# carsonswope/3d-beats

Hardware: AMD Instinct MI355X
Metric: classified Mpix/s on 848x480 depth frames (4 trees, depth 20); % of the bounding roofline level (roofline.bound; HBM: roofline.hbm_frac) (higher is better)
Workload: dtype f32

## Files before the change

3d-beats_amd/_lib.py:

```python
import ctypes
import os
import threading
import warnings

from . import _build

_c_int, _c_float, _c_void_p, _c_size_t = ctypes.c_int, ctypes.c_float, ctypes.c_void_p, ctypes.c_size_t

SIGNATURES = {
    "rdf_eval_forest": (_c_int, [_c_void_p, _c_int, _c_int, _c_int, _c_void_p, _c_int, _c_int, _c_int,
                                 _c_void_p, _c_int, _c_void_p, _c_int, _c_float, _c_void_p]),
    "rdf_eval_tree": (_c_int, [_c_void_p, _c_int, _c_int, _c_int, _c_void_p, _c_int, _c_int, _c_void_p,
                               _c_void_p]),
    "rdf_composite": (_c_int, [_c_void_p, _c_int, _c_int, _c_int, _c_void_p, _c_int, _c_void_p, _c_void_p,
                               _c_void_p]),
    "rdf_layered_run": (_c_int, [_c_void_p, _c_int, _c_int, _c_int, _c_void_p, _c_void_p, _c_void_p, _c_void_p, _c_void_p,
                                 _c_void_p, _c_void_p, _c_void_p, _c_void_p, _c_void_p, _c_int, _c_void_p, _c_void_p,
                                 _c_int, _c_float, _c_void_p]),
    "rdf_layered_run_hand": (_c_int, [_c_void_p, _c_int, _c_int, _c_int, _c_void_p, _c_void_p, _c_void_p, _c_void_p, _c_void_p,
                                      _c_void_p, _c_void_p, _c_void_p, _c_void_p, _c_void_p, _c_int, _c_void_p, _c_void_p,
                                      _c_int, _c_float, _c_int, _c_void_p, _c_int, _c_void_p, _c_void_p]),
    "rdf_layered_run_hand_batch": (_c_int, [_c_void_p, _c_int, _c_int, _c_int, _c_int, _c_void_p, _c_void_p, _c_void_p, _c_void_p,
                                            _c_void_p, _c_void_p, _c_void_p, _c_void_p, _c_void_p, _c_void_p, _c_int, _c_void_p,
                                            _c_void_p, _c_int, _c_float, _c_int, _c_void_p, _c_int, _c_void_p, _c_void_p]),
# ... 76 lines not shown
    "rdf_ipc_export": (_c_int, [_c_void_p, _c_void_p]),
    "rdf_ipc_open": (_c_int, [_c_void_p, _c_void_p]),
    "rdf_ipc_close": (_c_int, [_c_void_p]),
    "rdf_memcpy_device_async": (_c_int, [_c_void_p, _c_void_p, _c_size_t, _c_void_p]),
    "rdf_debug_fat_kernel": (_c_int, [_c_int, ctypes.c_uint64, _c_void_p, _c_void_p]),
    "rdf_debug_floor_i32": (_c_int, [_c_void_p, _c_void_p, _c_size_t, _c_void_p]),
    "rdf_debug_div_f32": (_c_int, [_c_void_p, _c_void_p, _c_void_p, _c_size_t, _c_void_p]),
    "rdf_set_lds_budget_bytes": (None, [_c_int]),
    "rdf_set_block_threads": (None, [_c_int]),
    "rdf_set_scheduler": (None, [_c_int]),
    "rdf_set_compaction": (None, [_c_int]),
    "rdf_set_halo": (None, [_c_int]),
    "rdf_set_lds_levels": (None, [_c_int]),
    "rdf_set_tree_waves": (None, [_c_int]),
    "rdf_set_stage_vec": (None, [_c_int]),
    "rdf_set_group": (None, [_c_int]),
    "rdf_set_layers_one_launch": (None, [_c_int]),
    "rdf_set_rows_per_wave": (None, [_c_int]),
    "rdf_set_force_exact": (None, [_c_int]),
    "rdf_set_last_level_table": (None, [_c_int]),
    "rdf_set_deep_from": (None, [_c_int]),
    "rdf_set_fold": (None, [_c_int]),
    "rdf_set_plain_levels": (None, [_c_int]),
    "rdf_event_create": (_c_int, [ctypes.POINTER(_c_void_p)]),
    "rdf_event_record": (_c_int, [_c_void_p, _c_void_p]),
    "rdf_event_synchronize": (_c_int, [_c_void_p]),
    "rdf_event_elapsed_ms": (_c_int, [_c_void_p, _c_void_p, ctypes.POINTER(_c_float)]),
    "rdf_event_destroy": (_c_int, [_c_void_p]),
    "rdf_stream_synchronize": (_c_int, [_c_void_p]),
    "rdf_abi_version": (_c_int, []),
    "rdf_build_id": (ctypes.c_char_p, []),
    "rdf_error_string": (ctypes.c_char_p, [_c_int]),
}

ABI_VERSION = 5


class StereoConfig(ctypes.Structure):
    _fields_ = [("fb16", ctypes.c_int32), ("fbp16", ctypes.c_int32), ("max_disparity", ctypes.c_int32),
                ("dot_threshold", ctypes.c_uint32), ("pattern_seed", ctypes.c_uint32), ("ambient", ctypes.c_int32),
                ("ir_noise_amp", ctypes.c_int32), ("census_margin", ctypes.c_int32), ("uniqueness", ctypes.c_int32),
                ("lr_max", ctypes.c_int32), ("dq_min", ctypes.c_int32)]


class DepthFilterConfig(ctypes.Structure):
    _fields_ = [(name, ctypes.c_int32) for name in ("spatial_radius", "spatial_delta", "temporal", "temporal_alpha", "temporal_delta",
# ... 152 lines not shown
```

3d-beats_amd/csrc/rdf_hip.hip:

```cpp

#include <hip/hip_runtime.h>
#include <stdint.h>
#include <stdio.h>
#include <stdlib.h>
#include <string.h>
#include <time.h>
#include <unistd.h>

#include <algorithm>
#include <array>
#include <atomic>
#include <mutex>
#include <utility>
#include <vector>

#include "../../include/rdf_hip.h"
#include "rdf_device.hpp"
#include "rdf_host_state.hpp"
#include "rdf_launch_plan.hpp"

namespace {

constexpr uint32_t kFlagLeftLeaf = 1u, kFlagRightLeaf = 2u, kFlagExact = 4u;
using rdf_host::kSchedSlots;
using rdf_host::kGraphSlots;

constexpr uint32_t kStealFrom = 2;
constexpr uint32_t kXcdQueuesFrom = 64;
__device__ unsigned int g_sched[kSchedSlots + kGraphSlots][kSchedWords];

__device__ __forceinline__ uint32_t child_flags(float l, float r)
{
    return ((l >= -1.0f && l < 0.0f) ? 0u : kFlagLeftLeaf) | ((r >= -1.0f && r < 0.0f) ? 0u : kFlagRightLeaf);
}

__device__ __forceinline__ bool int_offset_ok(float a)
{
    const uint32_t b = __float_as_uint(a);
    return (b << 1) == 0u || (((b >> 23) & 0xFFu) - 40u) <= 107u;
}

__device__ __forceinline__ uint32_t guarded_payload(uint32_t byte)
{
    return (byte & 0xFFu) | ((~byte & 0x80u) << 1);
}

__device__ __forceinline__ int thresh_to_int(float t)
{
    if (t != t) return -65535;
    const float c = fminf(fmaxf(__builtin_ceilf(t), -65535.0f), 65536.0f);
    return (int)c;
}
// ... 85 lines not shown
    const uint32_t role = NL > 1 ? blockIdx.x % NL : 0u;
    const uint32_t block_id = NL > 1 ? blockIdx.x / NL : blockIdx.x, n_blocks = NL > 1 ? gridDim.x / NL : gridDim.x;
    const EvalArgs &a = ka.l[role];
    extern __shared__ __align__(16) unsigned char lds_raw[];
    uint16_t *lds_tile = reinterpret_cast<uint16_t *>(lds_raw);
    uint4 *lds_nodes = reinterpret_cast<uint4 *>(lds_raw + a.lds_nodes_off);
    uint32_t *s_tile = reinterpret_cast<uint32_t *>(lds_raw + a.lds_mail_off);
    uint16_t *px_list = reinterpret_cast<uint16_t *>(lds_raw + a.lds_list_off);

    const int tid = threadIdx.x;
    const int lane = tid & 63;
    const int K = a.lds_levels;
    const uint32_t nodes_lds = (1u << K) - 1u;
    constexpr uint32_t kWaves = BLOCK / 64;
    const int rows_per_wave = a.rows_per_wave;
    const uint32_t wave = (uint32_t)tid >> 6;
    const uint32_t tw_T = TW ? (uint32_t)a.T : 1u;
    const uint32_t tw_row = TW ? wave / tw_T : 0u, tw_tree = TW ? wave - tw_row * tw_T : 0u;
    const uint32_t tile_rows = TW ? (kWaves / tw_T) * (uint32_t)rows_per_wave : kWaves * (uint32_t)rows_per_wave;

    const uint32_t lds_pitch = 1u << K;
    constexpr bool kLastLevelTable = PACKED && CMAX == 4 && !TW;
    constexpr bool kPlainLevels = PACKED && !STATS && !TW && !DEEP && NL == 1 && BLOCK == 512 && CMAX == 4 && GROUP == 4 && !COMPACT;
    bool last_from_table = false;
    if (kLastLevelTable && a.last_level) {
        const uint2 t = *reinterpret_cast<const uint2 *>(a.last_level + (((size_t)a.T << (a.D - 1)) << 2));
        last_from_table = t.x == 0u && t.y >= a.last_level_min;
    }
    constexpr int kDeepLast = CMAX == 4 ? 2 : 1;
    bool deep_on = false;
    if (DEEP && a.deep) {
        const uint2 t = *reinterpret_cast<const uint2 *>(a.deep + ((deep_total_lines(a.T, a.D, a.cpad) + 1u) << 3));
        deep_on = (uint32_t)a.deep_from >= t.x && t.y == 0u;
    }
    if (DEEP && deep_on) last_from_table = false;
    const int walk_levels = (DEEP && deep_on) ? a.deep_from : last_from_table ? a.D - 1 : a.D;
    for (uint32_t i = tid; i < (uint32_t)a.T * lds_pitch; i += BLOCK) {
        const uint32_t k = i >> K, h = i & (lds_pitch - 1u);
        if (h == 0u) {
            if (K > 0) lds_nodes[i] = make_uint4(0u, 0u, 0u, 0u);
            continue;
        }
        if (PACKED) {
            lds_nodes[i] = reinterpret_cast<const uint4 *>(a.packed16)[((size_t)k << a.D) + h];
        } else {
            const float *p = a.forest + ((size_t)k * (size_t)a.nodes + (h - 1u)) * (size_t)a.E;
// ... 21 lines not shown
        return (active && (!prev_active || prev != line)) ? 1u : 0u;
    };
    const char *depth_b = reinterpret_cast<const char *>(a.depth);
    const uint32_t xcc = (uint32_t)__builtin_amdgcn_s_getreg(20 | (31 << 11)) & 7u;
    const uint32_t q_static = a.q_static ? a.q_static : n_blocks;
    const uint32_t q_blocks = a.q_blocks ? a.q_blocks : n_blocks;
    const uint32_t queued = a.n_tiles > q_static ? a.n_tiles - q_static : 0u;

    struct TilePlace { uint32_t img, x0, y0, fold, col_shift; bool narrow; };
    auto place_tile = [&](uint32_t tile) -> TilePlace {
        const uint32_t tiles_wide = a.tiles_x * a.tiles_y;
        const uint32_t tiles_per_img = tiles_wide + a.tiles_y_n;
        TilePlace p;
        p.img = tile / tiles_per_img;
        const uint32_t trem = tile - p.img * tiles_per_img;
        p.narrow = trem >= tiles_wide;
        const uint32_t ty = p.narrow ? trem - tiles_wide : trem / a.tiles_x;
        const uint32_t tx = p.narrow ? a.tiles_x : trem - ty * a.tiles_x;
        p.fold = p.narrow ? a.fold : 1u;
        p.col_shift = p.narrow ? (a.fold == 4u ? 4u : 5u) : 6u;
        p.x0 = tx * 64u, p.y0 = ty * tile_rows * p.fold;
        return p;
    };
    auto rows_have_pixels = [&](const TilePlace &p, uint32_t first, uint32_t step, bool store_fails) -> bool {
        const uint32_t lane_col = (uint32_t)lane & ((1u << p.col_shift) - 1u), lane_row = (uint32_t)lane >> p.col_shift;
        const uint32_t lx = p.x0 + lane_col;
        const int y_last = min(a.Hl, (int)(p.y0 + tile_rows * p.fold)) - 1;
        const uint32_t img_boff = (p.img * a.per_img_d) << 1, img_loff = p.img * a.per_img_l;
        const uint32_t dy = step * p.fold;
        uint32_t ly = p.y0 + first * p.fold + lane_row;
        uint32_t seen = 0u;
        if ((int)lx < a.Wl) {
#pragma clang loop unroll(disable)
            for (uint32_t trow = first; trow < tile_rows; trow += 4u * step, ly += 4u * dy) {
                uint32_t i[4], d[4];
#pragma unroll
                for (uint32_t k = 0; k < 4u; ++k) {
                    const uint32_t y = (uint32_t)min((int)(ly + k * dy), y_last);
                    i[k] = img_loff + y * (uint32_t)a.Wl + lx;
                    d[k] = *reinterpret_cast<const uint16_t *>(
                        depth_b + (img_boff + ((__umul24(y * (uint32_t)a.r, (uint32_t)a.W) + lx * (uint32_t)a.r) << 1)));
                }
                if (a.filter_class != -1) {
                    uint32_t f[4];
#pragma unroll
                    for (uint32_t k = 0; k < 4u; ++k) f[k] = a.filter[i[k]];
#pragma unroll
                    for (uint32_t k = 0; k < 4u; ++k) d[k] = (int)f[k] == a.filter_class ? d[k] : 0u;
                }
#pragma unroll
                for (uint32_t k = 0; k < 4u; ++k) {
                    d[k] = (d[k] + 1u) & 0xFFFFu;
                    seen = max(seen, d[k]);
                    if (store_fails && d[k] <= 1u) a.labels[i[k]] = (uint16_t)kNoPixel;
                }
            }
        }
        return seen > 1u;
    };
    auto fill_tile = [&](const TilePlace &p) {
        const uint32_t lane_col = (uint32_t)lane & ((1u << p.col_shift) - 1u), lane_row = (uint32_t)lane >> p.col_shift;
        const int lx = (int)(p.x0 + lane_col);
#pragma clang loop vectorize(disable) unroll(disable)
        for (uint32_t trow = 0; trow < tile_rows; ++trow) {
            const int ly = (int)(p.y0 + trow * p.fold + lane_row);
            if (ly < a.Hl && lx < a.Wl) a.labels[p.img * a.per_img_l + (uint32_t)ly * (uint32_t)a.Wl + (uint32_t)lx] = (uint16_t)kNoPixel;
        }
    };
    auto pull_tile = [&](uint32_t after, uint32_t &q_empty) -> uint32_t {
        if (!a.sched) return after + n_blocks < a.n_tiles ? after + n_blocks : a.n_tiles;
        uint32_t t = a.n_tiles;
        if (q_static < kXcdQueuesFrom) {
            const uint32_t got = atomicAdd(a.sched, 1u);
            if (got < queued) t = q_static + got;
        } else {
            const uint32_t reach = (((block_id >> 3) & 15u) == 0u || queued >= 2u * q_static || a.q_helper) ? 7u : kStealFrom;
            for (uint32_t k = 0; k <= reach; ++k) {
                const uint32_t q = (xcc + k) & 7u;
                if ((q_empty >> q) & 1u) continue;
                const uint32_t lo = (uint32_t)(((unsigned long long)queued * q) >> 3);
                const uint32_t hi = (uint32_t)(((unsigned long long)queued * (q + 1u)) >> 3);
                const uint32_t got = lo < hi ? atomicAdd(a.sched + q * kSchedStride, 1u) : hi;
                if (lo < hi && got < hi - lo) { t = q_static + lo + got; break; }
                q_empty |= 1u << q;
            }
        }
        return t;
    };
    const bool more_tiles = a.sched ? queued != 0u : block_id + n_blocks < a.n_tiles;
    bool scout = !TW && a.sched && a.q_helper && wave == 0u;
    uint32_t q_empty = 0u;
    uint32_t tile = block_id;

    for (uint32_t it = 0;; ++it) {
        const bool own_tile = it == 0u && !(a.sched && a.q_helper);
        if (!own_tile && !more_tiles) break;
        if (TW) {
            if (!own_tile && tid == 0) s_tile[it & 1u] = pull_tile(tile, q_empty);
        } else {
            if (own_tile && a.check_empty) __syncthreads();
            if (scout || (own_tile && a.check_empty)) {
                uint32_t t = tile;
                q_empty = s_tile[6];
                for (;;) {
                    if (!own_tile) {
                        if (lane == 0) t = pull_tile(t, q_empty);
                        t = (uint32_t)__builtin_amdgcn_readfirstlane((int)t);
                    }
                    if (t >= a.n_tiles || !a.check_empty) break;
                    const TilePlace p = place_tile(t);
                    const bool any = (p.narrow ? a.tw_n : a.tw) <= 0 ||
                                     __any(rows_have_pixels(p, own_tile ? wave : 0u, own_tile ? kWaves : 1u, own_tile && a.fill_untouched));
                    if (own_tile) {
                        if (any && lane == 0) s_tile[2] = 1u;
                        break;
                    }
                    if (any) break;
                    if (a.fill_untouched) fill_tile(p);
                }
                if (!own_tile && lane == 0) {
                    s_tile[it & 1u] = t;
                    s_tile[6] = q_empty;
                }
            }
            scout = false;
        }
        __syncthreads();
        if (!own_tile) {
            tile = (uint32_t)__builtin_amdgcn_readfirstlane((int)s_tile[it & 1u]);
            if (!TW && tid == 0) s_tile[4u + ((it + 1u) & 1u)] = 0u;
        }
        if (tile >= a.n_tiles) break;
        if (!TW && own_tile && a.check_empty && s_tile[2] == 0u) {
            scout = wave == 0u;
            continue;
        }
        const TilePlace tp = place_tile(tile);
        const uint32_t img = tp.img;
        const bool narrow = tp.narrow;
        const uint32_t fold = tp.fold, col_shift = tp.col_shift;
        const uint32_t lane_col = (uint32_t)lane & ((1u << col_shift) - 1u), lane_row = (uint32_t)lane >> col_shift;
        const uint32_t x0 = tp.x0, y0 = tp.y0;
        const int lx = (int)(x0 + lane_col);
        const uint32_t img_boff = (img * a.per_img_d) << 1;
        const uint32_t img_loff = img * a.per_img_l;
        const int tx0 = (int)x0 * a.r - (narrow ? a.halo_xn : a.halo);
        const int ty0 = (int)y0 * a.r - a.halo;
        const int tw = narrow ? a.tw_n : a.tw, th = narrow ? a.th_n : a.th, twp = narrow ? a.twp_n : a.twp;
        const uint32_t stage_tw8 = narrow ? a.stage_tw8_n : a.stage_tw8, stage_magic = narrow ? a.stage_magic_n : a.stage_magic;

        const TileCtx pc = {depth_b + img_boff,
                            (uint32_t)tw * 2u, (uint32_t)th, (uint32_t)twp * 2u, (uint32_t)a.W * 2u, (uint32_t)a.H,
// ... 75 lines not shown
            my_rank[sub] = (uint32_t)__popcll(b & ((1ull << lane) - 1ull));
            my_valid |= ok ? 1u << sub : 0u;
        }
        uint32_t n_valid = 64u * tile_rows;
        if (compact) {
            __syncthreads();
            n_valid = 0u;
            uint32_t my_base[kMaxRowsPerWave];
            for (uint32_t row = 0; row < tile_rows; ++row) {
#pragma unroll
                for (int sub = 0; sub < kMaxRowsPerWave; ++sub)
                    if (row == (uint32_t)sub * kWaves + wave) my_base[sub] = n_valid;
                n_valid += s_cnt[row];
            }
#pragma unroll
            for (int sub = 0; sub < kMaxRowsPerWave; ++sub) {
                if (sub >= rows_per_wave) break;
                if ((my_valid >> sub) & 1u)
                    px_list[my_base[sub] + my_rank[sub]] = (uint16_t)((((uint32_t)sub * kWaves + wave) << 6) | (uint32_t)lane);
            }
            __syncthreads();
        }

        constexpr uint32_t kDone = 0x80000000u, kIdle = 0xFFFFFFFFu;
        auto add_leaf_pdf = [&](uint32_t hk, int tree, int c0, float (&pdf)[CMAX]) -> bool {
            if (STATS && c0 == 0)
                st_leaf += lines_of((int)hk < 0 && hk != kIdle, PACKED ? (hk & ~kDone) * (uint32_t)(a.cpad * 4) : ((hk & ~kDone) >> 1) * (uint32_t)a.E * 4u);
            if (!((int)hk < 0 && hk != kIdle)) return false;
            const uint32_t leaf = (hk & ~kDone) - 2u;
            if (PACKED) {
                const float4 *pp = reinterpret_cast<const float4 *>(a.packed_pdf) +
                    (((((size_t)tree) << a.D) + (leaf >> 1) + 1u) * 2u + (leaf & 1u)) * (size_t)(a.cpad >> 2) +
                    (size_t)(c0 >> 2);
#pragma unroll
                for (int c = 0; c < CMAX; c += 4) {
                    if (c0 + c < a.cpad) {
                        const float4 v = pp[c >> 2];
                        pdf[c] = pdf[c] + v.x; pdf[c + 1] = pdf[c + 1] + v.y;
                        pdf[c + 2] = pdf[c + 2] + v.z; pdf[c + 3] = pdf[c + 3] + v.w;
                    }
                }
            } else {
                const float *pp = a.forest +
                    ((size_t)tree * (size_t)a.nodes + (leaf >> 1)) * (size_t)a.E +
                    7 + (leaf & 1u) * a.C + c0;
#pragma unroll
                for (int c = 0; c < CMAX; c += 4) {
                    if (c0 + c + 3 < a.C) {
                        const f4u v = *reinterpret_cast<const f4u *>(pp + c);
                        pdf[c] = pdf[c] + v.x; pdf[c + 1] = pdf[c + 1] + v.y;
                        pdf[c + 2] = pdf[c + 2] + v.z; pdf[c + 3] = pdf[c + 3] + v.w;
                    } else {
#pragma unroll
                        for (int e = 0; e < 4; ++e)
                            if (c0 + c + e < a.C) pdf[c + e] = pdf[c + e] + pp[c + e];
                    }
                }
            }
            return true;
        };
        uint32_t tw_h = kIdle, tw_i = 0u;
        bool tw_valid = false;
        for (uint32_t first = TW ? (tw_row < tile_rows ? tw_row * 64u : n_valid) : wave * 64u; first < n_valid; first += BLOCK) {
            const uint32_t slot = first + (uint32_t)lane;
            uint32_t entry = slot;
            bool live = true;
            if (compact) {
                if (slot >= n_valid) {
                    if (!DEEP) continue;
                    live = false;
                }
                entry = px_list[live ? slot : first];
            }
            const int ly = (int)(y0 + (entry >> 6) * fold + ((entry & 63u) >> col_shift));
            const int px = (int)(x0 + (entry & ((1u << col_shift) - 1u)));
            if (!compact && (ly >= a.Hl || px >= a.Wl)) {
                if (!DEEP) continue;
                live = false;
            }
            const uint32_t i = img_loff + (uint32_t)ly * (uint32_t)a.Wl + (uint32_t)px;
            const int x = px * a.r, y = ly * a.r;
            const int xl = x - tx0, yl = y - ty0;
            bool skip = false;
            if (!compact && live && a.filter_class != -1) skip = (int)a.filter[i] != a.filter_class;
            uint32_t d = 0u;
            if (!skip && live) d = (uint32_t)tprobe_value(tprobe_issue(pc, (uint32_t)xl * 2u, (uint32_t)yl));
            if (!compact && live && (skip || d == 0u || d == kNoPixel)) {
                if (a.fill_untouched && (!TW || tw_tree == 0u)) a.labels[i] = (uint16_t)kNoPixel;
                if (!DEEP) continue;
                live = false;
            }
            if (DEEP && !live) d = 1u;
            const float df = (float)d;
            const float r0 = __builtin_amdgcn_rcpf(df);
            const float rcp = __builtin_fmaf(__builtin_fmaf(-df, r0, 1.0f), r0, r0);
            float rcp_s = rcp * (1.0f / kNumScale);
            const float df_s = df * kNumScale;
            uint32_t kx2 = ((uint32_t)xl - kMagicBits) * 2u;
            const uint32_t ky = (uint32_t)yl - kMagicBits;
            pin(kx2);

            float best = 0.0f;
            int best_c = 0;
            bool any_leaf = false;

            for (int c0 = 0; c0 < a.C || c0 == 0; c0 += CMAX) {
                float pdf[CMAX];
// ... 88 lines not shown
                                const int tk = min(kb + k, a.T - 1);
                                const float *p = a.forest + ((size_t)tk * (size_t)a.nodes + (hn[k] - 1u)) * (size_t)a.E;
                                if (STATS && c0 == 0) st_rec += lines_of((int)h[k] > 0, (hn[k] - 1u) * (uint32_t)a.E * 4u);
                                const f4u uv = *reinterpret_cast<const f4u *>(p);
                                const f3u tf = *reinterpret_cast<const f3u *>(p + 4);
                                n[k].ax = a.s * uv.x; n[k].ay = a.s * uv.y; n[k].bx = a.s * uv.z; n[k].by = a.s * uv.w;
                                set_threshold(n[k], thresh_to_int(tf.x));
                                n[k].flags = child_flags(tf.y, tf.z) | kFlagExact;
                            }
                        }

                        uint32_t ux[GROUP], uy[GROUP], vx[GROUP], vy[GROUP];
                        uint32_t fl = 0u;
#pragma unroll
                        for (int k = 0; k < GROUP; ++k) fl |= n[k].flags;
                        if (__any((fl & kFlagExact) != 0u)) {
                            const bool switch_mode = PACKED || in_lds;
                            if (switch_mode) set_round_nearest(df_e);
                            if (PACKED || in_lds) {
#pragma unroll
                                for (int k = 0; k < GROUP; ++k) {
                                    if (n[k].flags & kFlagExact) {
                                        const int tk = min(kb + k, a.T - 1);
                                        if (a.forest) {
                                            const float s_exact = (PACKED && a.info) ? a.info->scale : a.s;
                                            const float *p = a.forest +
                                                ((size_t)tk * (size_t)a.nodes + (hn[k] - 1u)) * (size_t)a.E;
                                            n[k].ax = s_exact * p[0]; n[k].ay = s_exact * p[1];
                                            n[k].bx = s_exact * p[2]; n[k].by = s_exact * p[3];
                                        } else {
                                            n[k].ax = n[k].ay = n[k].bx = n[k].by = 0.0f;
                                            if (a.stale_flag) __hip_atomic_store(a.stale_flag, 1u, __ATOMIC_RELAXED, __HIP_MEMORY_SCOPE_SYSTEM);
                                        }
                                    }
                                }
                            }
#pragma unroll
                            for (int k = 0; k < GROUP; ++k) {
                                const float den = (n[k].flags & kFlagExact) ? df_e : df_s;
                                ux[k] = (uint32_t)min(max(add_wrap(xl, floor_i32(n[k].ax / den)), -(1 << 30)), (1 << 30) - 1) * 2u;
                                uy[k] = (uint32_t)add_wrap(yl, floor_i32(n[k].ay / den));
                                vx[k] = (uint32_t)min(max(add_wrap(xl, floor_i32(n[k].bx / den)), -(1 << 30)), (1 << 30) - 1) * 2u;
                                vy[k] = (uint32_t)add_wrap(yl, floor_i32(n[k].by / den));
                            }
                            if (switch_mode) {
#pragma unroll
                                for (int k = 0; k < GROUP; ++k) { pin(ux[k]); pin(uy[k]); pin(vx[k]); pin(vy[k]); }
                                set_round_down(ux[0]);
                            }
                        } else {
#pragma unroll
                            for (int k = 0; k < GROUP; ++k) {
                                const f2 nu = {n[k].ax, n[k].ay};
                                const f2 nv = {n[k].bx, n[k].by};
                                const f2 r2 = {rcp_s, rcp_s};
// ... 274 lines not shown
                        any_leaf |= add_leaf_pdf(xch[(tw_row * tw_T + t) * 64u + (uint32_t)lane], (int)t, c0, pdf);
#pragma unroll
                    for (int c = 0; c < CMAX; ++c) {
                        if (c0 + c < a.C && pdf[c] > best) {
                            best = pdf[c];
                            best_c = c0 + c;
                        }
                    }
                }
                if (a.keep_if_no_leaf && !any_leaf) {
                    if (a.fill_untouched) a.labels[tw_i] = (uint16_t)kNoPixel;
                } else {
                    a.labels[tw_i] = (uint16_t)best_c;
                }
            }
        }
        if (!TW && more_tiles) {
            uint32_t before = 0u;
            if (lane == 0) before = atomicAdd(&s_tile[4u + (it & 1u)], 1u);
            scout = __builtin_amdgcn_readfirstlane((int)before) == 0;
        }
    }

    if (PACKED && a.info && a.stale_flag && block_id == n_blocks - 1u && tid == 0 && !a.q_helper) {
        if (a.info->generation != a.expect_gen)
            __hip_atomic_store(a.stale_flag, 1u, __ATOMIC_RELAXED, __HIP_MEMORY_SCOPE_SYSTEM);
    }

    if (a.sched && queued != 0u && tid == 0) {
        const unsigned int done = atomicAdd(a.sched + 8 * kSchedStride, 1u);
        if (done == q_blocks - 1u) {
            for (int q = 0; q < 9; ++q) atomicExch(a.sched + q * kSchedStride, 0u);
        }
    }

    if (STATS) {
        uint32_t c[8] = {st_px, st_lv, st_lf, st_lds, st_rec, st_leaf, st_far, st_blk};
#pragma unroll
        for (int i = 0; i < 8; ++i) {
            unsigned long long v = c[i];
            for (int o = 32; o > 0; o >>= 1) v += __shfl_down(v, o);
            if (lane == 0 && (i < 3 || a.stats_wide)) atomicAdd(a.stats + i, v);
        }
    }
}

__global__ __launch_bounds__(256) void k_pack(const float *forest, NodeRec16 *packed16, PackInfo *info,
                                              float *packed_pdf, LastLevelRec *last_level, unsigned int *last_level_unusable,
                                              uint4 *deep, int n_trees, int C, int cpad,
                                              size_t total_slots, int D, int E, float s, int force_exact, uint32_t generation)
{
    const size_t slot = (size_t)blockIdx.x * 256 + threadIdx.x;
    if (slot >= total_slots) return;
    const size_t tree = slot >> D, h = slot & (((size_t)1 << D) - 1);
    if (h == 0) {
        NodeRec16 z16 = {{0u, 0u, 0u, 0u}};
        packed16[slot] = z16;
        for (int c = 0; c < 2 * cpad; ++c) packed_pdf[slot * 2 * (size_t)cpad + c] = 0.f;
        if (tree == 0) {
            info->scale = s; info->magic = kPackMagic; info->generation = generation;
            info->n_trees = (uint32_t)n_trees; info->max_depth = (uint32_t)D; info->n_classes = (uint32_t)C;
        }
        if (deep && tree == 0) {
            uint4 *z = deep + (deep_total_lines(n_trees, D, cpad) << 3);
            for (int i = 0; i < 8; ++i) z[i] = make_uint4(0u, 0u, 0u, 0u);
        }
        return;
    }
// ... 903 lines not shown
    if (n == 0) return RDF_OK;
    if (!num || !den || !out) return RDF_ERR_NULL_PTR;
    hipLaunchKernelGGL(k_debug_div, dim3((unsigned)((n + 255) / 256)), dim3(256), 0,
                       reinterpret_cast<hipStream_t>(stream), num, den, out, n);
    return (int)hipGetLastError();
}

void rdf_set_lds_budget_bytes(int bytes) { g_lds_budget.value = bytes; }
void rdf_set_block_threads(int threads) { g_block_threads.value = threads; }
void rdf_set_scheduler(int mode) { g_sched_mode.value = mode; }
void rdf_set_compaction(int mode) { g_compaction.value = mode; }
void rdf_set_halo(int pixels) { g_halo.value = pixels; }
void rdf_set_group(int trees) { g_group.value = trees; }
void rdf_set_layers_one_launch(int on) { g_layers_one_launch.value = on; }
void rdf_set_lds_levels(int levels) { g_lds_levels.value = levels; }
void rdf_set_tree_waves(int mode) { g_tree_waves.value = mode; }
void rdf_set_stage_vec(int on) { g_stage_vec.value = on; }
void rdf_set_rows_per_wave(int rows) { g_rows_per_wave.value = rows; }
void rdf_set_force_exact(int on) { g_force_exact.value = on; }
void rdf_set_last_level_table(int on) { g_last_level_table.value = on; }
void rdf_set_deep_from(int level) { g_deep_from.value = level; }
void rdf_set_fold(int on) { g_fold.value = on; }
void rdf_set_plain_levels(int on) { g_plain_levels.value = on; }

int rdf_stream_create_with_reserved_cus(void **stream, int n_reserved)
{
    if (!stream || n_reserved < 1) return RDF_ERR_BAD_ARG;
    DeviceState *ds = nullptr;
    const int rc = current_device(&ds);
    if (rc != 0) return rc;
    const int cus = ds->cus.load(std::memory_order_relaxed);
    if (n_reserved >= cus) return RDF_ERR_BAD_ARG;
    const int words = (cus + 31) / 32;
    std::vector<uint32_t> mask((size_t)words, 0u);
    for (int cu = n_reserved; cu < cus; ++cu) mask[cu >> 5] |= 1u << (cu & 31);
    hipStream_t st;
    const hipError_t e = hipExtStreamCreateWithCUMask(&st, (uint32_t)words, mask.data());
    if (e != hipSuccess) return (int)e;
    *stream = st;
    return RDF_OK;
}
int rdf_stream_destroy(void *stream)
{
    const hipError_t e = hipStreamSynchronize(reinterpret_cast<hipStream_t>(stream));
    DeviceState *ds = nullptr;
    if (current_device(&ds) == 0) ds->drop_stream(stream);
// ... 30 lines not shown
    return RDF_OK;
}

int rdf_debug_kernel_launches(unsigned long long *out, int n, int reset)
{
    for (int i = 0; i < kNumForestKernels; ++i) {
        const unsigned long long v = reset ? g_kernel_launches[i].exchange(0, std::memory_order_relaxed)
                                           : g_kernel_launches[i].load(std::memory_order_relaxed);
        if (out && i < n) out[i] = v;
    }
    return kNumForestKernels;
}

int rdf_debug_kernel_key(int index, int key_out[9])
{
    if (index < 0 || index >= kNumForestKernels) return RDF_ERR_BAD_ARG;
    if (!key_out) return RDF_ERR_NULL_PTR;
    const KernelKey &k = kForestKernels[index];
    const int f[9] = {k.block, k.packed, k.cmax, k.stats, k.group, k.compact, k.nl, k.tw, k.deep};
    for (int i = 0; i < 9; ++i) key_out[i] = f[i];
    return RDF_OK;
}

int rdf_debug_sched_slots(int *stream_slots_in_use, int *graph_slots_used)
{
    DeviceState *ds = nullptr;
    if (current_device(&ds) != 0) return RDF_ERR_NO_DEVICE;
    ds->slots_in_use(stream_slots_in_use, graph_slots_used);
    return RDF_OK;
}

int rdf_device_malloc(void **ptr, size_t bytes)
{
    if (!ptr) return RDF_ERR_NULL_PTR;
    return (int)hipMalloc(ptr, bytes);
}
int rdf_device_free(void *ptr) { return (int)hipFree(ptr); }
int rdf_ipc_export(void *ptr, unsigned char handle_out[64])
{
    static_assert(sizeof(hipIpcMemHandle_t) == 64, "handle size");
    if (!ptr || !handle_out) return RDF_ERR_NULL_PTR;
    hipIpcMemHandle_t h;
    const hipError_t e = hipIpcGetMemHandle(&h, ptr);
    if (e != hipSuccess) return (int)e;
    memcpy(handle_out, &h, 64);
    return RDF_OK;
// ... 74 lines not shown
```

3d-beats_amd/csrc/rdf_launch_plan.hpp:

```cpp
#pragma once

#include <stdint.h>
#include <stdlib.h>
#include <string.h>

#include <algorithm>
#include <atomic>
#include <mutex>

#include "../../include/rdf_hip.h"
#include "rdf_host_state.hpp"

#ifdef __HIPCC__
#define RDF_HOST_DEVICE __host__ __device__
#else
#define RDF_HOST_DEVICE
#endif

namespace {

constexpr int kGroup = 4;
constexpr int kMaxRowsPerWave = 4;
constexpr int kDefaultLdsBudget = 32700;
constexpr int kDefaultLdsBudget512 = 54600;
// ... 74 lines not shown
    uint32_t stage_magic;
    uint32_t lds_xchg_off;
    uint32_t lds_nodes_off;
    uint32_t lds_mail_off;
    uint32_t lds_list_off;
    uint32_t lds_slab_off;
    const float *packed_pdf;
    const Vec16 *last_level;
    uint32_t last_level_min;
    const Vec16 *deep;
    int deep_from;
    int cpad;
    int filter_class;
    int check_empty;
    int keep_if_no_leaf;
    int fill_untouched;
    int plain_levels;
    float s;
    const PackInfo *info;
    uint32_t expect_gen;
    unsigned int *stale_flag;
    uint32_t q_static, q_blocks;
    int q_helper;
};

template <int NL>
struct EvalArgsN {
    EvalArgs l[NL];
};

struct Knob {
    const int unset;
    const char *const env;
    std::atomic<int> value;
    std::once_flag env_once;
    int env_set = 0, env_val = 0;
    Knob(int unset_, const char *env_) : unset(unset_), env(env_), value(unset_) {}
    int get(int dflt, bool *by_setter = nullptr)
    {
        const int v = value;
        if (by_setter) *by_setter = v > unset;
        if (v > unset) return v;
        if (!env) return dflt;
        std::call_once(env_once, [this]() {
            const char *s = getenv(env);
            if (s && *s) { env_set = 1; env_val = atoi(s); }
        });
        return env_set ? env_val : dflt;
    }
};
Knob g_compaction{-1, nullptr};
Knob g_group{0, nullptr};
Knob g_force_exact{0, nullptr};
Knob g_sched_mode{-1, nullptr};
Knob g_lds_budget{0, nullptr}, g_env_lds_budget{-1, "RDF_LDS_BUDGET"}, g_env_coop_lds_budget{-1, "RDF_COOP_LDS_BUDGET"};
Knob g_env_check_empty_small{-1, "RDF_CHECK_EMPTY_SMALL"};
Knob g_env_last_level_min_pct{-1, "RDF_LAST_LEVEL_MIN_PCT"};
Knob g_block_threads{0, "RDF_BLOCK"};
Knob g_rows_per_wave{0, "RDF_ROWS_PER_WAVE"};
Knob g_halo{-1, "RDF_HALO"};
Knob g_lds_levels{-1, "RDF_LDS_LEVELS"};
Knob g_tree_waves{-1, "RDF_TREE_WAVES"};
Knob g_stage_vec{-1, "RDF_STAGE_VEC"};
Knob g_layers_one_launch{-1, "RDF_LAYERS_ONE_LAUNCH"};
Knob g_fold{-1, "RDF_FOLD"};
Knob g_plain_levels{-1, "RDF_PLAIN_LEVELS"};
Knob g_deep_from{-1, "RDF_DEEP_FROM"};
Knob g_last_level_table{-1, "RDF_LAST_LEVEL_TABLE"};

int coop_lds_budget(int block)
{
    const int knob = g_lds_budget.get(0);
    const int v = knob > 0 ? knob : g_env_coop_lds_budget.get(0);
    if (v > 0) return v;
    return block == 512 ? 81920 - 65536 - 1024 : 40960 - 32768 - 1024;
}

int lds_budget(int block)
{
    const int knob = g_lds_budget.get(0);
    int b = knob > 0 ? knob : g_env_lds_budget.get(block == 512 ? kDefaultLdsBudget512 : kDefaultLdsBudget);
    if (b > 160 * 1024) b = 160 * 1024;
    if (b < 0) b = 0;
    return b;
}

using rdf_host::DeviceState;
using rdf_host::PackedState;

int sched_mode()
{
// ... 253 lines not shown
    a.T = q.n_trees; a.D = q.max_depth; a.C = q.n_classes; a.E = 7 + 2 * q.n_classes;
    a.nodes = (int)((1ll << q.max_depth) - 1);
    a.filter_class = q.filter_class;
    a.keep_if_no_leaf = q.keep_if_no_leaf;
    a.fill_untouched = q.fill_untouched;
    a.s = q.s;
    if (q.packed) {
        const size_t slots = (size_t)q.n_trees << q.max_depth;
        a.packed16 = reinterpret_cast<const NodeRec16 *>(q.packed);
        a.packed_pdf = reinterpret_cast<const float *>(a.packed16 + slots);
        a.cpad = classes_padded(q.n_classes);
        if (ps.exact_nodes > 0 && !q.forest) return RDF_ERR_NULL_PTR;
        a.s = ps.scale;
        a.info = reinterpret_cast<const PackInfo *>(ps.info_dev);
        a.expect_gen = ps.generation;
        a.stale_flag = stale_flag_dev;
    }
    const bool compaction = g_compaction.get(1) != 0;
    const Geometry &g = plan->g = choose_geometry(q, a.Wl, a.Hl, device_cus, ps, compaction);
    if (g.n_tiles >= (1ll << 31)) return RDF_ERR_TOO_LARGE;
    a.fold = g.fold; a.tiles_x = g.tiles_x; a.tiles_y = g.tiles_y; a.tiles_y_n = g.tiles_y_n;
    a.n_tiles = (uint32_t)g.n_tiles; a.rows_per_wave = g.rpw;
    a.plain_levels = g_plain_levels.get(1) != 0;
    a.check_empty = (g.big || q.r > 1) ? 1 : g_env_check_empty_small.get(0);
    plan->compact_launch = q.packed && !q.stats && q.filter_class != -1 && compaction;
    plan->lds_bytes = lay_out_lds(q, g, plan->compact_launch, a);
    plan->deep = g.deep_from_wanted > 0;
    plan->packed = q.packed != nullptr; plan->stats = q.stats != nullptr;
    return RDF_OK;
}

struct KernelKey {
    int block; bool packed; int cmax; bool stats; int group; bool compact; int nl; bool tw; bool deep;
};
constexpr bool operator==(const KernelKey &a, const KernelKey &b)
{
    return a.block == b.block && a.packed == b.packed && a.cmax == b.cmax && a.stats == b.stats && a.group == b.group &&
           a.compact == b.compact && a.nl == b.nl && a.tw == b.tw && a.deep == b.deep;
}

constexpr KernelKey kForestKernels[] = {
    {256, true, 4, false, 1, false, 1, false, false},  {512, true, 4, false, 1, false, 1, false, false},
    {256, true, 4, false, 2, false, 1, false, false},  {512, true, 4, false, 2, false, 1, false, false},
    {256, true, 4, false, 3, false, 1, false, false},  {512, true, 4, false, 3, false, 1, false, false},
    {256, true, 4, false, 4, false, 1, false, false},  {512, true, 4, false, 4, false, 1, false, false},
    {256, true, 8, false, 1, false, 1, false, false},  {512, true, 8, false, 1, false, 1, false, false},
// ... 67 lines not shown
```

include/rdf_hip.h:

```cpp
#ifndef RDF_HIP_H
#define RDF_HIP_H

#include <stddef.h>
#include <stdint.h>

#ifdef __cplusplus
extern "C" {
#endif

#define RDF_ABI_VERSION 5

#define RDF_OK 0
#define RDF_ERR_BAD_ARG (-1)
#define RDF_ERR_NULL_PTR (-2)
#define RDF_ERR_TOO_LARGE (-3)
#define RDF_ERR_NO_DEVICE (-4)
#define RDF_ERR_BUILD (-5)
#define RDF_ERR_CAPTURE (-6)
#define RDF_ERR_STALE (-7)

int rdf_eval_forest(const uint16_t *depth, int n_img, int dim_x, int dim_y,
                    const float *forest, int n_trees, int max_depth, int n_classes,
                    const uint16_t *filter, int filter_class,
                    uint16_t *labels_out, int labels_reduce, float scale_factor, void *stream);
// ... 148 lines not shown
int rdf_train_update_pixels(const uint16_t *depth, int n_img, int dim_x, int dim_y, int level, int max_depth,
                            int n_classes, int32_t *nodes_by_pixel, const float *tree, void *stream);

int rdf_fill_u16(uint16_t *dst, size_t n, uint16_t value, void *stream);

int rdf_stream_create_with_reserved_cus(void **stream, int n_reserved);
int rdf_stream_destroy(void *stream);
int rdf_stream_capture_id(void *stream, unsigned long long *capture_id);
int rdf_graph_slots_release(unsigned long long capture_id);
int rdf_debug_sched_slots(int *stream_slots_in_use, int *graph_slots_used);
int rdf_device_malloc(void **ptr, size_t bytes);
int rdf_device_free(void *ptr);
int rdf_ipc_export(void *ptr, unsigned char handle_out[64]);
int rdf_ipc_open(const unsigned char handle[64], void **ptr_out);
int rdf_ipc_close(void *ptr);
int rdf_memcpy_device_async(void *dst, const void *src, size_t bytes, void *stream);
int rdf_debug_fat_kernel(int n_workgroups, unsigned long long spin_ticks, unsigned long long *t_start, void *stream);
int rdf_debug_floor_i32(const float *in, int32_t *out, size_t n, void *stream);
int rdf_debug_div_f32(const float *num, const float *den, float *out, size_t n, void *stream);

int rdf_debug_host_overhead(unsigned long long out[5], int reset);
int rdf_debug_kernel_launches(unsigned long long *out, int n, int reset);
int rdf_debug_kernel_key(int index, int key_out[9]);

void rdf_set_lds_budget_bytes(int bytes);
void rdf_set_block_threads(int threads);
void rdf_set_compaction(int mode);
void rdf_set_scheduler(int mode);
void rdf_set_rows_per_wave(int rows);
void rdf_set_halo(int pixels);
void rdf_set_tree_waves(int mode);
void rdf_set_lds_levels(int levels);
void rdf_set_group(int trees);
void rdf_set_layers_one_launch(int on);
void rdf_set_stage_vec(int on);
void rdf_set_force_exact(int on);
void rdf_set_last_level_table(int on);

void rdf_set_deep_from(int level);
void rdf_set_fold(int on);
void rdf_set_plain_levels(int on);
int rdf_event_create(void **event);
int rdf_event_record(void *event, void *stream);
int rdf_event_synchronize(void *event);
int rdf_event_elapsed_ms(void *start, void *stop, float *ms);
int rdf_event_destroy(void *event);
int rdf_stream_synchronize(void *stream);

int rdf_abi_version(void);
const char *rdf_build_id(void);
const char *rdf_error_string(int code);

#ifdef __cplusplus
}
#endif
#endif
```

Baseline: 14530.

## Add opt-in per-tile pixel dealing to pack sparse tiles into dense waves

Adds a per-tile compaction mode for the plain-levels kernel. It counts valid pixels per row with ballots and, when enough rows can be saved, deals the valid pixels densely across waves so that no lane idles on empty pixels. The scout also marks tiles where every pixel is valid so those skip the check. Rarely used arguments (filter, forest, info, stale_flag) are now read straight from the kernarg segment to reduce register pressure. The compaction defaults to off (margin 0), so the default path only picks up the kernarg reads and the extra full-tile check.

```diff
diff --git a/3d-beats_amd/_lib.py b/3d-beats_amd/_lib.py
--- a/3d-beats_amd/_lib.py
+++ b/3d-beats_amd/_lib.py
@@ -122,6 +122,8 @@
     "rdf_set_deep_from": (None, [_c_int]),
     "rdf_set_fold": (None, [_c_int]),
     "rdf_set_plain_levels": (None, [_c_int]),
+    "rdf_set_tile_compaction": (None, [_c_int]),
+    "rdf_debug_compacted_tiles": (_c_int, [_c_void_p, _c_int]),
     "rdf_event_create": (_c_int, [ctypes.POINTER(_c_void_p)]),
     "rdf_event_record": (_c_int, [_c_void_p, _c_void_p]),
     "rdf_event_synchronize": (_c_int, [_c_void_p]),
diff --git a/3d-beats_amd/csrc/rdf_hip.hip b/3d-beats_amd/csrc/rdf_hip.hip
--- a/3d-beats_amd/csrc/rdf_hip.hip
+++ b/3d-beats_amd/csrc/rdf_hip.hip
@@ -28,6 +28,7 @@
 constexpr uint32_t kStealFrom = 2;
 constexpr uint32_t kXcdQueuesFrom = 64;
 __device__ unsigned int g_sched[kSchedSlots + kGraphSlots][kSchedWords];
+__device__ unsigned long long g_compacted_tiles;
 
 __device__ __forceinline__ uint32_t child_flags(float l, float r)
 {
@@ -159,6 +160,12 @@
     const uint32_t lds_pitch = 1u << K;
     constexpr bool kLastLevelTable = PACKED && CMAX == 4 && !TW;
     constexpr bool kPlainLevels = PACKED && !STATS && !TW && !DEEP && NL == 1 && BLOCK == 512 && CMAX == 4 && GROUP == 4 && !COMPACT;
+    auto cold = [&]() {
+        auto *p = (const __attribute__((address_space(4))) EvalArgsN<NL> *)__builtin_amdgcn_kernarg_segment_ptr();
+        asm volatile("" : "+s"(p));
+        return p;
+    };
+#define RDF_COLD_ARG(field) (kPlainLevels ? cold()->l[0].field : a.field)
     bool last_from_table = false;
     if (kLastLevelTable && a.last_level) {
         const uint2 t = *reinterpret_cast<const uint2 *>(a.last_level + (((size_t)a.T << (a.D - 1)) << 2));
@@ -226,6 +233,7 @@
         p.x0 = tx * 64u, p.y0 = ty * tile_rows * p.fold;
         return p;
     };
+    bool rows_all_pixels = false;
     auto rows_have_pixels = [&](const TilePlace &p, uint32_t first, uint32_t step, bool store_fails) -> bool {
         const uint32_t lane_col = (uint32_t)lane & ((1u << p.col_shift) - 1u), lane_row = (uint32_t)lane >> p.col_shift;
         const uint32_t lx = p.x0 + lane_col;
@@ -234,7 +242,9 @@
         const uint32_t dy = step * p.fold;
         uint32_t ly = p.y0 + first * p.fold + lane_row;
         uint32_t seen = 0u;
+        uint32_t low = 0u;
         if ((int)lx < a.Wl) {
+            low = 0xFFFFu;
 #pragma clang loop unroll(disable)
             for (uint32_t trow = first; trow < tile_rows; trow += 4u * step, ly += 4u * dy) {
                 uint32_t i[4], d[4];
@@ -248,7 +258,7 @@
                 if (a.filter_class != -1) {
                     uint32_t f[4];
 #pragma unroll
-                    for (uint32_t k = 0; k < 4u; ++k) f[k] = a.filter[i[k]];
+                    for (uint32_t k = 0; k < 4u; ++k) f[k] = RDF_COLD_ARG(filter)[i[k]];
 #pragma unroll
                     for (uint32_t k = 0; k < 4u; ++k) d[k] = (int)f[k] == a.filter_class ? d[k] : 0u;
                 }
@@ -256,10 +266,12 @@
                 for (uint32_t k = 0; k < 4u; ++k) {
                     d[k] = (d[k] + 1u) & 0xFFFFu;
                     seen = max(seen, d[k]);
+                    if constexpr (kPlainLevels) low = min(low, d[k]);
                     if (store_fails && d[k] <= 1u) a.labels[i[k]] = (uint16_t)kNoPixel;
                 }
             }
         }
+        if constexpr (kPlainLevels) rows_all_pixels = low > 1u;
         return seen > 1u;
     };
     auto fill_tile = [&](const TilePlace &p) {
@@ -296,6 +308,7 @@
     uint32_t q_empty = 0u;
     uint32_t tile = block_id;
 
+    constexpr uint32_t kDealt = 0x80000000u;
     for (uint32_t it = 0;; ++it) {
         const bool own_tile = it == 0u && !(a.sched && a.q_helper);
         if (!own_tile && !more_tiles) break;
@@ -311,6 +324,7 @@
                         if (lane == 0) t = pull_tile(t, q_empty);
                         t = (uint32_t)__builtin_amdgcn_readfirstlane((int)t);
                     }
+                    rows_all_pixels = false;
                     if (t >= a.n_tiles || !a.check_empty) break;
                     const TilePlace p = place_tile(t);
                     const bool any = (p.narrow ? a.tw_n : a.tw) <= 0 ||
@@ -322,16 +336,22 @@
                     if (any) break;
                     if (a.fill_untouched) fill_tile(p);
                 }
+                const bool full = kPlainLevels && __all(rows_all_pixels);
                 if (!own_tile && lane == 0) {
-                    s_tile[it & 1u] = t;
+                    s_tile[it & 1u] = t | (full ? kDealt : 0u);
                     s_tile[6] = q_empty;
                 }
             }
             scout = false;
         }
         __syncthreads();
+        bool tile_full = false;
         if (!own_tile) {
             tile = (uint32_t)__builtin_amdgcn_readfirstlane((int)s_tile[it & 1u]);
+            if constexpr (kPlainLevels) {
+                tile_full = (tile & kDealt) != 0u;
+                tile &= ~kDealt;
+            }
             if (!TW && tid == 0) s_tile[4u + ((it + 1u) & 1u)] = 0u;
         }
         if (tile >= a.n_tiles) break;
@@ -453,6 +473,80 @@
             __syncthreads();
         }
 
+        auto row_depth = [&](uint32_t l, uint32_t trow) -> uint32_t {
+            const uint32_t px = x0 + (l & ((1u << col_shift) - 1u)), ly = y0 + trow * fold + (l >> col_shift);
+            const uint32_t d = *(const __attribute__((address_space(3))) uint16_t *)(uintptr_t)(
+                __umul24(ly * (uint32_t)a.r - (uint32_t)ty0, pc.twp2) + (px * (uint32_t)a.r - (uint32_t)tx0) * 2u);
+            return ((int)ly < a.Hl && (int)px < a.Wl) ? d : 0u;
+        };
+        auto deal_group = [&](uint32_t g) -> uint32_t {
+            uint32_t l = (uint32_t)lane;
+            pin(l);
+            const uint32_t want = g * 64u + l;
+            uint32_t base = 0u;
+            uint32_t my_row = 0u, my_k = 0u, my_lo = 0u, my_hi = 0u;
+#pragma clang loop unroll(disable)
+            for (uint32_t trow = 0; trow < tile_rows; trow += 4u) {
+                uint32_t d[4];
+#pragma unroll
+                for (uint32_t k = 0; k < 4u; ++k) d[k] = row_depth(l, trow + k);
+#pragma unroll
+                for (uint32_t k = 0; k < 4u; ++k) {
+                    const unsigned long long m = __ballot(d[k] != 0u && d[k] != kNoPixel);
+                    const uint32_t cnt = (uint32_t)__popcll(m), k_in = want - base;
+                    const bool mine = k_in < cnt;
+                    my_row = mine ? trow + k : my_row;
+                    my_k = mine ? k_in : my_k;
+                    my_lo = mine ? (uint32_t)m : my_lo;
+                    my_hi = mine ? (uint32_t)(m >> 32) : my_hi;
+                    base += cnt;
+                }
+            }
+            uint32_t c = (uint32_t)__popc(my_lo);
+            bool up = my_k >= c;
+            uint32_t w = up ? my_hi : my_lo, pos = up ? 32u : 0u;
+            my_k = up ? my_k - c : my_k;
+#pragma unroll
+            for (uint32_t s = 16u; s >= 1u; s >>= 1) {
+                c = (uint32_t)__popc(w & ((1u << s) - 1u));
+                up = my_k >= c;
+                my_k = up ? my_k - c : my_k;
+                w = up ? w >> s : w;
+                pos += up ? s : 0u;
+            }
+            return (my_row << 6) | pos;
+        };
+        if constexpr (kPlainLevels) {
+            if ((a.tile_compaction & 0xFF) != 0 && a.filter_class == -1 && tw > 0 && !tile_full) {
+                uint32_t n = 0u, rows = 0u;
+#pragma clang loop unroll(disable)
+                for (uint32_t trow = 0; trow < tile_rows; trow += 4u) {
+                    uint32_t d[4];
+#pragma unroll
+                    for (uint32_t k = 0; k < 4u; ++k) d[k] = row_depth((uint32_t)lane, trow + k);
+#pragma unroll
+                    for (uint32_t k = 0; k < 4u; ++k) {
+                        const unsigned long long m = __ballot(d[k] != 0u && d[k] != kNoPixel);
+                        n += (uint32_t)__popcll(m);
+                        rows += m != 0ull ? 1u : 0u;
+                    }
+                }
+                if (((n + 63u) >> 6) + (uint32_t)(a.tile_compaction & 0xFF) <= rows) {
+                    n_valid = n | kDealt;
+                    if (a.fill_untouched) {
+                        for (uint32_t trow = wave; trow < tile_rows; trow += kWaves) {
+                            const uint32_t ly = y0 + trow * fold + lane_row;
+                            const uint32_t d = row_depth((uint32_t)lane, trow);
+                            if ((int)ly < a.Hl && lx < a.Wl && (d == 0u || d == kNoPixel))
+                                a.labels[img_loff + ly * (uint32_t)a.Wl + (uint32_t)lx] = (uint16_t)kNoPixel;
+                        }
+                    }
+                    if ((a.tile_compaction & kCountCompactedTiles) != 0 && tid == 0)
+                        __hip_atomic_fetch_add(&g_compacted_tiles, 1ull, __ATOMIC_RELAXED, __HIP_MEMORY_SCOPE_AGENT);
+                }
+            }
+        }
+
         constexpr uint32_t kDone = 0x80000000u, kIdle = 0xFFFFFFFFu;
         auto add_leaf_pdf = [&](uint32_t hk, int tree, int c0, float (&pdf)[CMAX]) -> bool {
             if (STATS && c0 == 0)
@@ -492,7 +586,7 @@
         };
         uint32_t tw_h = kIdle, tw_i = 0u;
         bool tw_valid = false;
-        for (uint32_t first = TW ? (tw_row < tile_rows ? tw_row * 64u : n_valid) : wave * 64u; first < n_valid; first += BLOCK) {
+        for (uint32_t first = TW ? (tw_row < tile_rows ? tw_row * 64u : n_valid) : wave * 64u; first < (kPlainLevels ? n_valid & ~kDealt : n_valid); first += BLOCK) {
             const uint32_t slot = first + (uint32_t)lane;
             uint32_t entry = slot;
             bool live = true;
@@ -503,6 +597,12 @@
                 }
                 entry = px_list[live ? slot : first];
             }
+            if constexpr (kPlainLevels) {
+                if ((n_valid & kDealt) != 0u) {
+                    entry = deal_group(first >> 6);
+                    if (slot >= (n_valid & ~kDealt)) continue;
+                }
+            }
             const int ly = (int)(y0 + (entry >> 6) * fold + ((entry & 63u) >> col_shift));
             const int px = (int)(x0 + (entry & ((1u << col_shift) - 1u)));
             if (!compact && (ly >= a.Hl || px >= a.Wl)) {
@@ -513,7 +613,7 @@
             const int x = px * a.r, y = ly * a.r;
             const int xl = x - tx0, yl = y - ty0;
             bool skip = false;
-            if (!compact && live && a.filter_class != -1) skip = (int)a.filter[i] != a.filter_class;
+            if (!compact && live && a.filter_class != -1) skip = (int)RDF_COLD_ARG(filter)[i] != a.filter_class;
             uint32_t d = 0u;
             if (!skip && live) d = (uint32_t)tprobe_value(tprobe_issue(pc, (uint32_t)xl * 2u, (uint32_t)yl));
             if (!compact && live && (skip || d == 0u || d == kNoPixel)) {
@@ -648,15 +748,15 @@
                                 for (int k = 0; k < GROUP; ++k) {
                                     if (n[k].flags & kFlagExact) {
                                         const int tk = min(kb + k, a.T - 1);
-                                        if (a.forest) {
-                                            const float s_exact = (PACKED && a.info) ? a.info->scale : a.s;
-                                            const float *p = a.forest +
+                                        if (RDF_COLD_ARG(forest)) {
+                                            const float s_exact = (PACKED && RDF_COLD_ARG(info)) ? RDF_COLD_ARG(info)->scale : a.s;
+                                            const float *p = RDF_COLD_ARG(forest) +
                                                 ((size_t)tk * (size_t)a.nodes + (hn[k] - 1u)) * (size_t)a.E;
                                             n[k].ax = s_exact * p[0]; n[k].ay = s_exact * p[1];
                                             n[k].bx = s_exact * p[2]; n[k].by = s_exact * p[3];
                                         } else {
                                             n[k].ax = n[k].ay = n[k].bx = n[k].by = 0.0f;
-                                            if (a.stale_flag) __hip_atomic_store(a.stale_flag, 1u, __ATOMIC_RELAXED, __HIP_MEMORY_SCOPE_SYSTEM);
+                                            if (RDF_COLD_ARG(stale_flag)) __hip_atomic_store(RDF_COLD_ARG(stale_flag), 1u, __ATOMIC_RELAXED, __HIP_MEMORY_SCOPE_SYSTEM);
                                         }
                                     }
                                 }
@@ -977,7 +1077,14 @@
         }
     }
 
-    if (PACKED && a.info && a.stale_flag && block_id == n_blocks - 1u && tid == 0 && !a.q_helper) {
+    if constexpr (kPlainLevels) {
+        if (block_id == n_blocks - 1u && tid == 0 && !a.q_helper) {
+            const PackInfo *const info_l = RDF_COLD_ARG(info);
+            unsigned int *const flag_l = RDF_COLD_ARG(stale_flag);
+            if (info_l && flag_l && info_l->generation != RDF_COLD_ARG(expect_gen))
+                __hip_atomic_store(flag_l, 1u, __ATOMIC_RELAXED, __HIP_MEMORY_SCOPE_SYSTEM);
+        }
+    } else if (PACKED && a.info && a.stale_flag && block_id == n_blocks - 1u && tid == 0 && !a.q_helper) {
         if (a.info->generation != a.expect_gen)
             __hip_atomic_store(a.stale_flag, 1u, __ATOMIC_RELAXED, __HIP_MEMORY_SCOPE_SYSTEM);
     }
@@ -999,6 +1106,7 @@
         }
     }
 }
+#undef RDF_COLD_ARG
 
 __global__ __launch_bounds__(256) void k_pack(const float *forest, NodeRec16 *packed16, PackInfo *info,
                                               float *packed_pdf, LastLevelRec *last_level, unsigned int *last_level_unusable,
@@ -1948,6 +2056,7 @@
 void rdf_set_deep_from(int level) { g_deep_from.value = level; }
 void rdf_set_fold(int on) { g_fold.value = on; }
 void rdf_set_plain_levels(int on) { g_plain_levels.value = on; }
+void rdf_set_tile_compaction(int on) { g_tile_compaction.value = on; }
 
 int rdf_stream_create_with_reserved_cus(void **stream, int n_reserved)
 {
@@ -2024,6 +2133,21 @@
     return RDF_OK;
 }
 
+int rdf_debug_compacted_tiles(unsigned long long *count, int reset)
+{
+    g_count_compacted_tiles.store(1, std::memory_order_relaxed);
+    hipError_t e = hipDeviceSynchronize();
+    unsigned long long v = 0;
+    if (e == hipSuccess) e = hipMemcpyFromSymbol(&v, HIP_SYMBOL(g_compacted_tiles), sizeof(v));
+    if (e == hipSuccess && reset) {
+        const unsigned long long zero = 0;
+        e = hipMemcpyToSymbol(HIP_SYMBOL(g_compacted_tiles), &zero, sizeof(zero));
+    }
+    if (e != hipSuccess) return (int)e;
+    if (count) *count = v;
+    return RDF_OK;
+}
+
 int rdf_debug_sched_slots(int *stream_slots_in_use, int *graph_slots_used)
 {
     DeviceState *ds = nullptr;
diff --git a/3d-beats_amd/csrc/rdf_launch_plan.hpp b/3d-beats_amd/csrc/rdf_launch_plan.hpp
--- a/3d-beats_amd/csrc/rdf_launch_plan.hpp
+++ b/3d-beats_amd/csrc/rdf_launch_plan.hpp
@@ -120,7 +120,9 @@
     unsigned int *stale_flag;
     uint32_t q_static, q_blocks;
     int q_helper;
-};
+    int tile_compaction;
+};
+constexpr int kCountCompactedTiles = 0x100;
 
 template <int NL>
 struct EvalArgsN {
@@ -163,8 +165,11 @@
 Knob g_layers_one_launch{-1, "RDF_LAYERS_ONE_LAUNCH"};
 Knob g_fold{-1, "RDF_FOLD"};
 Knob g_plain_levels{-1, "RDF_PLAIN_LEVELS"};
+Knob g_tile_compaction{-1, "RDF_TILE_COMPACTION"};
 Knob g_deep_from{-1, "RDF_DEEP_FROM"};
 Knob g_last_level_table{-1, "RDF_LAST_LEVEL_TABLE"};
+
+std::atomic<int> g_count_compacted_tiles{0};
 
 int coop_lds_budget(int block)
 {
@@ -464,6 +469,9 @@
     a.fold = g.fold; a.tiles_x = g.tiles_x; a.tiles_y = g.tiles_y; a.tiles_y_n = g.tiles_y_n;
     a.n_tiles = (uint32_t)g.n_tiles; a.rows_per_wave = g.rpw;
     a.plain_levels = g_plain_levels.get(1) != 0;
+    const int deal_margin = g_tile_compaction.get(0);
+    a.tile_compaction = (deal_margin < 0 ? 0 : deal_margin > 255 ? 255 : deal_margin) |
+                        (g_count_compacted_tiles.load(std::memory_order_relaxed) ? kCountCompactedTiles : 0);
     a.check_empty = (g.big || q.r > 1) ? 1 : g_env_check_empty_small.get(0);
     plan->compact_launch = q.packed && !q.stats && q.filter_class != -1 && compaction;
     plan->lds_bytes = lay_out_lds(q, g, plan->compact_launch, a);
diff --git a/include/rdf_hip.h b/include/rdf_hip.h
--- a/include/rdf_hip.h
+++ b/include/rdf_hip.h
@@ -194,6 +194,7 @@
 int rdf_debug_host_overhead(unsigned long long out[5], int reset);
 int rdf_debug_kernel_launches(unsigned long long *out, int n, int reset);
 int rdf_debug_kernel_key(int index, int key_out[9]);
+int rdf_debug_compacted_tiles(unsigned long long *count, int reset);
 
 void rdf_set_lds_budget_bytes(int bytes);
 void rdf_set_block_threads(int threads);
@@ -212,6 +213,7 @@
 void rdf_set_deep_from(int level);
 void rdf_set_fold(int on);
 void rdf_set_plain_levels(int on);
+void rdf_set_tile_compaction(int on);
 int rdf_event_create(void **event);
 int rdf_event_record(void *event, void *stream);
 int rdf_event_synchronize(void *event);
```

Measured after the change: 14520 (median of 2 runs). No clear change (-0.1%).
